# martenlienen/bsi

Measured on AMD Instinct MI355X. Metric: images/sec BSI.sample k=128 (DiT, 3x32x32), higher is better.
Workload: dtype bf16

## Files before the change

bsi_amd/csrc/dit_ops.hip:

```cpp
#include <math.h>

#include "common.h"
#include "dit_ops.h"

namespace {

constexpr int TPB = 256;

__global__ void silu_bf16_kernel(const float* __restrict__ pre, size_t n, __bf16* __restrict__ out) {
    for (size_t i = (size_t)blockIdx.x * blockDim.x + threadIdx.x; i < n; i += (size_t)gridDim.x * blockDim.x)
        out[i] = (__bf16)silu_f(pre[i]);
}

__global__ void cast_bf16_kernel(const float* __restrict__ in, int ld_in, int rows, int cols, __bf16* __restrict__ out, int ld) {
    const int r = blockIdx.y;
    const float* ir = in + (size_t)r * ld_in;
    __bf16* orow = out + (size_t)r * ld;
    for (int c = (blockIdx.x * blockDim.x + threadIdx.x) * 4; c < ld; c += gridDim.x * blockDim.x * 4) {
        float v[4];
#pragma unroll
        for (int k = 0; k < 4; ++k) v[k] = (c + k < cols) ? ir[c + k] : 0.0f;
        if (c + 3 < ld) {
            u32x2 w;
            w[0] = pack_bf16x2(v[0], v[1]);
// ... 185 lines not shown
        const float rstd = 1.0f / sqrtf(wave_sum(q) / (float)d + eps);
        __bf16* orow = out + (size_t)r * d;
#pragma unroll
        for (int i = 0; i < VPL; ++i) {
            const int c = i * 64 + lane;
            if (c < d4) {
                f32x4 y;
#pragma unroll
                for (int k = 0; k < 4; ++k) y[k] = (R.v[i][k] - mean) * rstd;
                const f32x4 a = tab[2][c];
                const f32x4 b = tab[3][c];
#pragma unroll
                for (int k = 0; k < 4; ++k) y[k] = __fmaf_rn(b[k] + 1.0f, y[k], a[k]);
                u32x2 w;
                w[0] = pack_bf16x2(y[0], y[1]);
                w[1] = pack_bf16x2(y[2], y[3]);
                reinterpret_cast<u32x2*>(orow)[c] = w;
            }
        }
    };
    Row A, B;
    if (row >= M) return;
    load(row, A);
    while (true) {
        if (row + stride < M) load(row + stride, B);
        finish(row, A);
        row += stride;
        if (row >= M) break;
        if (row + stride < M) load(row + stride, A);
        finish(row, B);
        row += stride;
        if (row >= M) break;
    }
}

__global__ void fourier_features_kernel(const float* __restrict__ x, size_t total, int C, int inner, int nmin,
                                        int nfreq, float* __restrict__ out) {
    for (size_t idx = (size_t)blockIdx.x * blockDim.x + threadIdx.x; idx < total; idx += (size_t)gridDim.x * blockDim.x) {
        const size_t in_i = idx % inner;
        const size_t oc = idx / inner;
        const float v = x[idx];
        float* o = out + (oc * nfreq * 2) * inner + in_i;
        for (int n = 0; n < nfreq; ++n) {
            const float coef = 6.283185307179586f * (float)(1 << (nmin + n));
            o[(size_t)(n * 2 + 0) * inner] = sinf(__fmaf_rn(coef, v, 0.0f));
            o[(size_t)(n * 2 + 1) * inner] = sinf(__fmaf_rn(coef, v, 1.5707963267948966f));
        }
    }
}

__global__ void dit_prologue_kernel(const float* __restrict__ mu, const float* __restrict__ c_in, int coef_stride, int B,
                                    int C, int H, int W, int ps, int nmin, int nfreq, int kpad, __bf16* __restrict__ out) {
    const int HW = H * W;
    const size_t total = (size_t)B * HW;
    const int Cin = C + C * nfreq * 2;
    const int nw = W / ps;
    const int tokens = (H / ps) * nw;
    const int K = ps * ps * Cin;
    for (size_t idx = (size_t)blockIdx.x * blockDim.x + threadIdx.x; idx < total; idx += (size_t)gridDim.x * blockDim.x) {
        const int b = (int)(idx / HW);
        const int pix = (int)(idx % HW);
        const int h = pix / W, w = pix % W;
        const float ci = c_in ? c_in[(size_t)b * coef_stride] : 1.0f;
        const int tok = (h / ps) * nw + (w / ps);
        const int intra = (h % ps) * ps + (w % ps);
        __bf16* o = out + ((size_t)b * tokens + tok) * kpad + intra * Cin;
        for (int c = 0; c < C; ++c) {
            float v = mu[((size_t)b * C + c) * HW + pix];
            if (c_in) v = __fmul_rn(ci, v);
            o[c] = (__bf16)v;
            for (int n = 0; n < nfreq; ++n) {
                const float coef = 6.283185307179586f * (float)(1 << (nmin + n));
                o[C + (c * nfreq + n) * 2 + 0] = (__bf16)sinf(__fmaf_rn(coef, v, 0.0f));
                o[C + (c * nfreq + n) * 2 + 1] = (__bf16)sinf(__fmaf_rn(coef, v, 1.5707963267948966f));
            }
        }
        if (intra == ps * ps - 1) {
            __bf16* z = out + ((size_t)b * tokens + tok) * kpad;
            for (int c = K; c < kpad; ++c) z[c] = (__bf16)0.0f;
        }
    }
}

template <int VPL, bool WLDS>
__global__ void dit_final_kernel(const float* __restrict__ x, int Mtok, int d, int P, const float* __restrict__ ln_w,
                                 const float* __restrict__ ln_b, const float* __restrict__ dec_w,
                                 const float* __restrict__ dec_b, int C, int H, int W, int ps,
                                 const float* __restrict__ mu, const float* __restrict__ c_skip,
                                 const float* __restrict__ c_out, int coef_stride, const __bf16* __restrict__ delta,
                                 const float* __restrict__ gate, int gate_rows, int gate_stride,
                                 float* __restrict__ out) {
    extern __shared__ __attribute__((aligned(16))) float wsm[];
    const int d4 = d >> 2;
    if constexpr (WLDS) {
        for (int i = threadIdx.x; i < P * d4; i += blockDim.x)
            reinterpret_cast<f32x4*>(wsm)[i] = reinterpret_cast<const f32x4*>(dec_w)[i];
        __syncthreads();
    }
    const int lane = threadIdx.x & 63;
    const int wpb = blockDim.x >> 6;
    const int nw = W / ps;
    const int tokens = (H / ps) * nw;
    const int HW = H * W;
    constexpr int FR = 4;
    for (int row0 = (blockIdx.x * wpb + (threadIdx.x >> 6)) * FR; row0 < Mtok; row0 += gridDim.x * wpb * FR) {
        f32x4 v[FR][VPL];
        float s[FR], q[FR];
#pragma unroll
        for (int r = 0; r < FR; ++r) {
            const int row = row0 + r < Mtok ? row0 + r : Mtok - 1;
            const float* xr = x + (size_t)row * d;
            const int b_idx = row / tokens;
            s[r] = 0.f;
#pragma unroll
            for (int i = 0; i < VPL; ++i) {
                const int c = i * 64 + lane;
                v[r][i] = (c < d4) ? reinterpret_cast<const f32x4*>(xr)[c] : f32x4{0.f, 0.f, 0.f, 0.f};
                if (delta && c < d4) {
                    const u32x2 dw = reinterpret_cast<const u32x2*>(delta + (size_t)row * d)[c];
                    const f32x4 g = reinterpret_cast<const f32x4*>(gate + (size_t)(b_idx % gate_rows) * gate_stride)[c];
                    v[r][i][0] = __fmaf_rn(g[0], __uint_as_float(dw[0] << 16), v[r][i][0]);
                    v[r][i][1] = __fmaf_rn(g[1], __uint_as_float(dw[0] & 0xffff0000u), v[r][i][1]);
                    v[r][i][2] = __fmaf_rn(g[2], __uint_as_float(dw[1] << 16), v[r][i][2]);
                    v[r][i][3] = __fmaf_rn(g[3], __uint_as_float(dw[1] & 0xffff0000u), v[r][i][3]);
                }
                s[r] += (v[r][i][0] + v[r][i][1]) + (v[r][i][2] + v[r][i][3]);
            }
        }
#pragma unroll
        for (int m = 32; m > 0; m >>= 1)
#pragma unroll
            for (int r = 0; r < FR; ++r) s[r] += __shfl_xor(s[r], m, 64);
#pragma unroll
        for (int r = 0; r < FR; ++r) {
            const float mean = s[r] / (float)d;
            s[r] = mean;
            q[r] = 0.f;
#pragma unroll
            for (int i = 0; i < VPL; ++i) {
                const int c = i * 64 + lane;
                if (c < d4) {
#pragma unroll
                    for (int k = 0; k < 4; ++k) {
                        const float dd = v[r][i][k] - mean;
                        q[r] = __fmaf_rn(dd, dd, q[r]);
                    }
                }
            }
        }
#pragma unroll
        for (int m = 32; m > 0; m >>= 1)
#pragma unroll
            for (int r = 0; r < FR; ++r) q[r] += __shfl_xor(q[r], m, 64);
#pragma unroll
        for (int i = 0; i < VPL; ++i) {
            const int c = i * 64 + lane;
            if (c < d4) {
                const f32x4 a = reinterpret_cast<const f32x4*>(ln_w)[c];
                const f32x4 bb = reinterpret_cast<const f32x4*>(ln_b)[c];
#pragma unroll
                for (int r = 0; r < FR; ++r) {
                    const float rstd = 1.0f / sqrtf(q[r] / (float)d + 1e-5f);
#pragma unroll
                    for (int k = 0; k < 4; ++k) v[r][i][k] = __fmaf_rn((v[r][i][k] - s[r]) * rstd, a[k], bb[k]);
                }
            }
        }
        float mine[FR] = {0.f, 0.f, 0.f, 0.f};
        for (int o0 = 0; o0 < P; o0 += 4) {
            float acc[FR][4];
#pragma unroll
            for (int r = 0; r < FR; ++r)
#pragma unroll
                for (int u = 0; u < 4; ++u) acc[r][u] = 0.f;
#pragma unroll
            for (int u = 0; u < 4; ++u) {
                const int o = o0 + u < P ? o0 + u : P - 1;
#pragma unroll
                for (int i = 0; i < VPL; ++i) {
                    const int c = i * 64 + lane;
                    if (c < d4) {
                        const f32x4 wv = WLDS ? reinterpret_cast<const f32x4*>(wsm + (size_t)o * d)[c]
                                              : reinterpret_cast<const f32x4*>(dec_w + (size_t)o * d)[c];
#pragma unroll
                        for (int r = 0; r < FR; ++r)
#pragma unroll
                            for (int k = 0; k < 4; ++k) acc[r][u] = __fmaf_rn(v[r][i][k], wv[k], acc[r][u]);
                    }
                }
            }
#pragma unroll
            for (int m = 32; m > 0; m >>= 1)
#pragma unroll
                for (int r = 0; r < FR; ++r)
#pragma unroll
                    for (int u = 0; u < 4; ++u) acc[r][u] += __shfl_xor(acc[r][u], m, 64);
#pragma unroll
            for (int u = 0; u < 4; ++u)
                if (o0 + u < P && lane == o0 + u) {
#pragma unroll
                    for (int r = 0; r < FR; ++r) mine[r] = acc[r][u] + dec_b[o0 + u];
                }
        }
        if (lane < P) {
            const int intra = lane / C, ch = lane % C;
#pragma unroll
            for (int r = 0; r < FR; ++r) {
                const int row = row0 + r;
                if (row >= Mtok) break;
                const int b_idx = row / tokens, tok = row % tokens;
                const int th = tok / nw, tw = tok % nw;
                const int hh = th * ps + intra / ps, ww = tw * ps + intra % ps;
                const size_t gi = ((size_t)b_idx * C + ch) * HW + (size_t)hh * W + ww;
                float rr = mine[r];
                if (c_skip) {
                    const float cs = c_skip[(size_t)b_idx * coef_stride], co = c_out[(size_t)b_idx * coef_stride];
                    rr = __fmaf_rn(co, mine[r], __fmul_rn(cs, mu[gi]));
                }
                out[gi] = rr;
            }
        }
    }
}

}

#define S(stream) reinterpret_cast<hipStream_t>(stream)

extern "C" int bsi_cast_rows_bf16(const float* in, int ld_in, int rows, int cols, void* out, int ld_out,
                                  bsi_stream_t stream) {
    BSI_CHECK_ARG(in && out && rows > 0 && cols > 0 && ld_in >= cols && ld_out >= cols && ld_out % 4 == 0,
                  "bsi_cast_rows_bf16: bad args rows=%d cols=%d ld_in=%d ld_out=%d", rows, cols, ld_in, ld_out);
    int gx = (ld_out / 4 + TPB - 1) / TPB;
    if (gx > 16) gx = 16;
    hipLaunchKernelGGL(cast_bf16_kernel, dim3(gx, rows), dim3(TPB), 0, S(stream), in, ld_in, rows, cols,
                       reinterpret_cast<__bf16*>(out), ld_out);
    BSI_CHECK_LAUNCH("bsi_cast_bf16");
    return BSI_OK;
}

extern "C" int bsi_cast_bf16(const float* in, int rows, int cols, void* out, int ld_out, bsi_stream_t stream) {
    return bsi_cast_rows_bf16(in, cols, rows, cols, out, ld_out, stream);
}

extern "C" int bsi_silu_bf16(const float* pre, size_t n, void* out, bsi_stream_t stream) {
    BSI_CHECK_ARG(pre && out && n > 0, "bsi_silu_bf16: bad args");
    size_t g = (n + TPB - 1) / TPB;
    if (g > 4096) g = 4096;
    hipLaunchKernelGGL(silu_bf16_kernel, dim3((int)g), dim3(TPB), 0, S(stream), pre, n, reinterpret_cast<__bf16*>(out));
    BSI_CHECK_LAUNCH("bsi_silu_bf16");
    return BSI_OK;
}

extern "C" int bsi_fourier_features(const float* x, int outer, int C, int inner, int n_min, int n_max, float* out,
                                    bsi_stream_t stream) {
    BSI_CHECK_ARG(x && out && outer > 0 && C > 0 && inner > 0 && n_max >= n_min && n_min >= 0 && n_max < 31,
                  "bsi_fourier_features: bad args");
    const size_t total = (size_t)outer * C * inner;
    size_t g = (total + TPB - 1) / TPB;
    if (g > 8192) g = 8192;
    hipLaunchKernelGGL(fourier_features_kernel, dim3((int)g), dim3(TPB), 0, S(stream), x, total, C, inner, n_min,
                       n_max - n_min + 1, out);
    BSI_CHECK_LAUNCH("bsi_fourier_features");
    return BSI_OK;
}

extern "C" int bsi_nyquist_embed(const float* t, int rows, const float* scale, const float* bias, int size,
                                 float* out_f32, void* out_bf16, bsi_stream_t stream) {
    BSI_CHECK_ARG(t && scale && bias && rows > 0 && size > 0 && (out_f32 || out_bf16), "bsi_nyquist_embed: bad args");
    int gx = (size + TPB - 1) / TPB;
    hipLaunchKernelGGL(nyquist_kernel, dim3(gx, rows), dim3(TPB), 0, S(stream), t, rows, scale, bias, size, out_f32,
                       reinterpret_cast<__bf16*>(out_bf16));
    BSI_CHECK_LAUNCH("bsi_nyquist_embed");
    return BSI_OK;
}

int bsi_resid_ln_modulate_drop(float* x, int M, int d, float eps, const void* delta, const float* gate,
                               const float* shift, const float* scale, int mod_rows, int mod_stride, int tokens,
                               const float* ln_w, const float* ln_b, void* out_bf16, DropCfg dc, bsi_stream_t stream,
                               float* x_out, float* stats, const void* delta0, const float* gate0, int write_x, DropCfg mdc,
                               void* maskw) {
    BSI_CHECK_ARG(x && M > 0 && d > 0 && d % 4 == 0 && d <= 2048, "bsi_resid_ln_modulate: bad args M=%d d=%d", M, d);
    BSI_CHECK_ARG(out_bf16 || delta, "bsi_resid_ln_modulate: nothing to do");
    BSI_CHECK_ARG((shift == nullptr) == (scale == nullptr), "bsi_resid_ln_modulate: shift and scale go together");
    BSI_CHECK_ARG((delta == nullptr) == (gate == nullptr), "bsi_resid_ln_modulate: delta and gate go together");
    BSI_CHECK_ARG(!(shift || gate) || (mod_rows > 0 && tokens > 0 && mod_stride % 4 == 0),
                  "bsi_resid_ln_modulate: bad modulation table");
    BSI_CHECK_ARG((ln_w == nullptr) == (ln_b == nullptr), "bsi_resid_ln_modulate: ln weight and bias go together");
    BSI_CHECK_ARG((delta0 == nullptr) == (gate0 == nullptr) && (!delta0 || delta), "bsi_resid_ln_modulate: an older update needs its gate and a newer update");
    BSI_CHECK_ARG(write_x || (delta && out_bf16 && !x_out), "bsi_resid_ln_modulate: write_x = 0 needs an update and an output");
    BSI_CHECK_ARG(!(maskw && mdc.thr) || (d > 256 && d <= 1024 && out_bf16), "bsi_resid_ln_modulate: mask words ride on the d <= 1024 instance");
    const __bf16* dl0 = reinterpret_cast<const __bf16*>(delta0);
    const int wpb = TPB / 64;
    dim3 grid((M + wpb - 1) / wpb);
    __bf16* o = reinterpret_cast<__bf16*>(out_bf16);
    const __bf16* dl = reinterpret_cast<const __bf16*>(delta);
    if (g_bsi_ln_stream_cus > 0 && d > 256 && d <= 1024 && shift && o && mod_rows == 1 && !ln_w && !dc.thr && !x_out && !stats &&
        !(maskw && mdc.thr)) {
        static int per_cu = 0;
        if (per_cu == 0) {
            int n = 0;
            if (hipOccupancyMaxActiveBlocksPerMultiprocessor(&n, ln_modulate_stream_kernel<4>, TPB, 0) != hipSuccess || n < 1) n = 2;
            if (const char* e = getenv("BSI_LN_STREAM_WGS")) n = atoi(e) > 0 ? atoi(e) : n;
            per_cu = n;
        }
        int g = g_bsi_ln_stream_cus * per_cu;
        if (g > (int)grid.x) g = (int)grid.x;
// ... 5 lines not shown
    if (d <= 256)
        hipLaunchKernelGGL(ln_modulate_kernel<1>, grid, dim3(TPB), 0, S(stream), x, M, d, eps, shift, scale, mod_rows,
                           mod_stride, tokens, ln_w, ln_b, dl, gate, o, dc, x_out, stats, dl0, gate0, write_x);
    else if (d <= 1024 && maskw && mdc.thr)
        hipLaunchKernelGGL((ln_modulate_kernel<4, true>), grid, dim3(TPB), 0, S(stream), x, M, d, eps, shift, scale, mod_rows,
                           mod_stride, tokens, ln_w, ln_b, dl, gate, o, dc, x_out, stats, dl0, gate0, write_x, mdc,
                           reinterpret_cast<unsigned long long*>(maskw));
    else if (d <= 1024)
        hipLaunchKernelGGL(ln_modulate_kernel<4>, grid, dim3(TPB), 0, S(stream), x, M, d, eps, shift, scale, mod_rows,
                           mod_stride, tokens, ln_w, ln_b, dl, gate, o, dc, x_out, stats, dl0, gate0, write_x);
    else
        hipLaunchKernelGGL(ln_modulate_kernel<8>, grid, dim3(TPB), 0, S(stream), x, M, d, eps, shift, scale, mod_rows,
                           mod_stride, tokens, ln_w, ln_b, dl, gate, o, dc, x_out, stats, dl0, gate0, write_x);
    BSI_CHECK_LAUNCH("bsi_resid_ln_modulate");
    return BSI_OK;
}

extern "C" int bsi_resid2_ln_modulate(float* x, int M, int d, float eps, const void* delta0, const float* gate0, const void* delta,
                                      const float* gate, int write_x, const float* shift, const float* scale, int mod_rows,
                                      int mod_stride, int tokens, void* out_bf16, bsi_stream_t stream) {
    return bsi_resid_ln_modulate_drop(x, M, d, eps, delta, gate, shift, scale, mod_rows, mod_stride, tokens, nullptr, nullptr,
                                      out_bf16, DropCfg{}, stream, nullptr, nullptr, delta0, gate0, write_x);
}

extern "C" int bsi_resid_ln_modulate(float* x, int M, int d, float eps, const void* delta, const float* gate,
                                     const float* shift, const float* scale, int mod_rows, int mod_stride, int tokens,
                                     const float* ln_w, const float* ln_b, void* out_bf16, bsi_stream_t stream) {
    return bsi_resid_ln_modulate_drop(x, M, d, eps, delta, gate, shift, scale, mod_rows, mod_stride, tokens, ln_w, ln_b,
                                      out_bf16, DropCfg{}, stream);
}

__global__ void dropout_mask_kernel(DropCfg dc, unsigned rows, unsigned cols, uint8_t* __restrict__ out) {
    const size_t n = (size_t)rows * cols;
    for (size_t i = (size_t)blockIdx.x * blockDim.x + threadIdx.x; i < n; i += (size_t)gridDim.x * blockDim.x) {
        const unsigned r = (unsigned)(i / cols), c = (unsigned)(i % cols);
        out[i] = drop_keep_rc(dc, drop_row(dc, r), c) ? 1 : 0;
    }
}

extern "C" int bsi_dropout_mask(float p, unsigned long long seed, unsigned site, unsigned rows, unsigned cols, uint8_t* out,
                                bsi_stream_t stream) {
    BSI_CHECK_ARG(out && rows > 0 && cols > 0 && p >= 0.f && p < 1.f, "bsi_dropout_mask: bad args");
    size_t g = ((size_t)rows * cols + TPB - 1) / TPB;
    if (g > 4096) g = 4096;
    hipLaunchKernelGGL(dropout_mask_kernel, dim3((int)g), dim3(TPB), 0, S(stream), make_drop(p, seed, site), rows, cols, out);
    BSI_CHECK_LAUNCH("bsi_dropout_mask");
    return BSI_OK;
}

extern "C" int bsi_ln_modulate(const float* x, int M, int d, float eps, const float* shift, const float* scale,
                               int mod_rows, int mod_stride, int tokens, const float* ln_w, const float* ln_b,
                               void* out_bf16, bsi_stream_t stream) {
    BSI_CHECK_ARG(out_bf16, "bsi_ln_modulate: null output");
    return bsi_resid_ln_modulate(const_cast<float*>(x), M, d, eps, nullptr, nullptr, shift, scale, mod_rows, mod_stride,
                                 tokens, ln_w, ln_b, out_bf16, stream);
}

int bsi_dit_prologue_launch(const float* mu, const float* c_in, int coef_stride, int B, int C, int H, int W, int ps,
                            int nmin, int nfreq, int kpad, void* out, hipStream_t s) {
    const size_t total = (size_t)B * H * W;
    size_t g = (total + TPB - 1) / TPB;
    if (g > 8192) g = 8192;
    hipLaunchKernelGGL(dit_prologue_kernel, dim3((int)g), dim3(TPB), 0, s, mu, c_in, coef_stride, B, C, H, W, ps, nmin,
                       nfreq, kpad, reinterpret_cast<__bf16*>(out));
    BSI_CHECK_LAUNCH("bsi_dit_prologue");
    return BSI_OK;
}

int bsi_dit_final_launch(const float* x, int Mtok, int d, int P, const float* ln_w, const float* ln_b,
                         const float* dec_w, const float* dec_b, int C, int H, int W, int ps, const float* mu,
                         const float* c_skip, const float* c_out, int coef_stride, const void* delta, const float* gate,
                         int gate_rows, int gate_stride, float* out, hipStream_t s) {
    size_t lds = (size_t)P * d * sizeof(float);
    if (P > 64) {
        bsi_set_error("bsi_dit_final: decoder P=%d unsupported (needs patch*patch*C <= 64)", P);
        return BSI_EINVAL;
    }
    const bool wlds = lds <= 128 * 1024;
    if (!wlds) lds = 0;
    const int wpb = TPB / 64;
    int grid = (Mtok + wpb * 4 - 1) / (wpb * 4);
    if (grid < 1) grid = 1;
    if (grid > 2048) grid = 2048;
#define LAUNCH_FINAL(V)                                                                                              \
    do {                                                                                                             \
        auto kern = wlds ? dit_final_kernel<V, true> : dit_final_kernel<V, false>;                                   \
        (void)hipFuncSetAttribute(reinterpret_cast<const void*>(kern), hipFuncAttributeMaxDynamicSharedMemorySize, (int)lds); \
        hipLaunchKernelGGL(kern, dim3(grid), dim3(TPB), lds, s, x, Mtok, d, P, ln_w, ln_b, dec_w, dec_b, C, H, W, ps, \
                           mu, c_skip, c_out, coef_stride, reinterpret_cast<const __bf16*>(delta), gate,             \
                           gate_rows > 0 ? gate_rows : 1, gate_stride, out);                                         \
    } while (0)
    if (d <= 256) LAUNCH_FINAL(1);
    else if (d <= 1024) LAUNCH_FINAL(4);
    else LAUNCH_FINAL(8);
#undef LAUNCH_FINAL
    BSI_CHECK_LAUNCH("bsi_dit_final");
    return BSI_OK;
}
```

bsi_amd/_native.py:

```python
import ctypes as C
import os

import torch

_HERE = os.path.dirname(os.path.abspath(__file__))
LIB_PATH = os.environ.get("BSI_HIP_LIB") or os.path.join(_HERE, "lib", "libbsi_hip.so")

_lib = None


class BSIParams(C.Structure):
    _fields_ = [("lambda_0", C.c_float), ("alpha_M", C.c_float), ("alpha_R", C.c_float),
                ("ln_low", C.c_float), ("delta", C.c_float)]


class GemmArgs(C.Structure):
    _fields_ = [("A", C.c_void_p), ("W", C.c_void_p), ("bias", C.c_void_p), ("out", C.c_void_p),
                ("M", C.c_int), ("N", C.c_int), ("K", C.c_int),
                ("lda", C.c_int), ("ldw", C.c_int), ("ldo", C.c_int), ("epilogue", C.c_int),
                ("gate", C.c_void_p), ("gate_rows", C.c_int), ("gate_stride", C.c_int),
                ("tokens", C.c_int), ("pos", C.c_void_p), ("aux", C.c_void_p), ("out2", C.c_void_p), ("colsum_rows", C.c_void_p)]


class CastDesc(C.Structure):
# ... 172 lines not shown
    "bsi_attention_fwd": (_i, [_vp, _i, _i, _i, _i, _i, _vp, _i, _vp]),
    "bsi_attention_fwd_lse": (_i, [_vp, _i, _i, _i, _i, _i, _vp, _i, _vp, _vp]),
    "bsi_attention_bwd": (_i, [_vp, _i, _vp, _vp, _i, _vp, _i, _i, _i, _i, _vp, _i, _vp]),
    "bsi_attention_bwd_long": (_i, [_vp, _i, _vp, _vp, _i, _vp, _i, _i, _i, _i, _vp, _i, _vp]),
    "bsi_gate_bwd": (_i, [_vp, _vp, _vp, _vp, _i, _vp, _i, _i, _i, _i, _vp, _vp]),
    "bsi_ln_mod_bwd": (_i, [_vp, _vp, _vp, _i, _vp, _vp, _i, _vp, _i, _i, _i, _f, _vp]),
    "bsi_ln_gate_bwd": (_i, [_vp, _vp, _vp, _vp, _i, _vp, _vp, _i, _vp, _vp, _vp, _i, _vp, _i, _vp, _i, _i, _i, _vp]),
    "bsi_silu_bwd_bf16": (_i, [_vp, _vp, _sz, _vp, _vp]),
    "bsi_cast_transpose_bf16": (_i, [_vp, _i, _i, _vp, _i, _vp]),
    "bsi_cast_batch_tiles": (_i, [_i, _i, _i]),
    "bsi_cast_batch_bf16": (_i, [_vp, _i, _i, _vp]),
    "bsi_cast_rows_bf16": (_i, [_vp, _i, _i, _i, _vp, _i, _vp]),
    "bsi_silu_bf16": (_i, [_vp, _sz, _vp, _vp]),
    "bsi_dit_tape_bytes": (_sz, [C.POINTER(DitConfig), _i]),
    "bsi_dit_backward_workspace_bytes": (_sz, [C.POINTER(DitConfig), _i]),
    "bsi_dit_train_forward": (_i, [C.POINTER(DitConfig), C.POINTER(DitWeights), _i, _vp, _vp, _vp, _vp, _vp, _vp, _vp,
                                   _f, C.c_ulonglong, _vp]),
    "bsi_dit_backward": (_i, [C.POINTER(DitConfig), C.POINTER(DitWeights), C.POINTER(DitWeightsT), C.POINTER(DitGrads), _i,
                              _vp, _vp, _vp, _vp, _f, C.c_ulonglong, _vp]),
    "bsi_dropout_mask": (_i, [_f, C.c_ulonglong, C.c_uint, C.c_uint, C.c_uint, _vp, _vp]),
    "bsi_attention_dropout_words": (_i, [_f, C.c_ulonglong, C.c_uint, _i, _vp, _vp]),
    "bsi_attention_fwd_dropout": (_i, [_vp, _i, _i, _i, _i, _i, _vp, _i, _vp, _f, C.c_ulonglong, C.c_uint, _vp, _vp]),
    "bsi_attention_bwd_dropout": (_i, [_vp, _i, _vp, _vp, _i, _vp, _i, _i, _i, _i, _vp, _i, _f, C.c_ulonglong, C.c_uint, _vp, _vp]),
    "bsi_dit_backward_set_events": (_i, [_vp, _i]),
    "bsi_dit_train_forward_set_gates": (_i, [_vp, _i]),
    "bsi_sqnorm_workspace_bytes": (_sz, []),
    "bsi_grad_sqnorm": (_i, [_vp, _sz, _vp, _vp, _vp]),
    "bsi_clip_adamw_ema": (_i, [_vp, _vp, _vp, _vp, _vp, _sz, _vp, _f, _f, _f, _f, _f, _f, _f, _i, _f, _vp]),
    "bsi_conv_nhwc_bf16": (_i, [C.POINTER(ConvArgs), _vp]),
    "bsi_conv_weight_pack": (_i, [_vp, _i, _i, _i, _i, _i, _i, _vp, _vp]),
    "bsi_conv_weight_pack_t": (_i, [_vp, _i, _i, _i, _i, _vp, _vp]),
    "bsi_conv_weight_pack_batch": (_i, [_vp, _i, _i, _vp]),
    "bsi_conv_wgrad_workspace_bytes": (C.c_size_t, [_i, _i, _i, _i, _i]),
    "bsi_conv_wgrad_nhwc_bf16": (_i, [_vp, _i, _vp, _vp, _vp, _i, _i, _i, _i, _i, _i, _i, _vp, _i, _vp, _vp]),
    "bsi_conv_wgrad_bias_nhwc_bf16": (_i, [_vp, _i, _vp, _vp, _vp, _i, _i, _i, _i, _i, _i, _i, _vp, _vp, _i, _vp, _vp]),
    "bsi_conv_wgrad_unpack": (_i, [_vp, _i, _i, _i, _i, _i, _i, _i, _vp, _vp]),
    "bsi_groupnorm_nhwc": (_i, [_vp, _i, _vp, _i, _i, _i, _vp, _vp, _f, _i, _vp, _vp, _vp]),
    "bsi_groupnorm_stats_nhwc": (_i, [_vp, _i, _vp, _i, _i, _i, _vp, _vp, _f, _i, _vp, _vp, _vp, _vp]),
    "bsi_groupnorm_apply_nhwc": (_i, [_vp, _i, _vp, _vp, _i, _vp, _i, _i, _vp, _vp, _f, _i, _vp, _vp, _vp, _vp]),
    "bsi_groupnorm_bwd_nhwc": (_i, [_vp, _vp, _i, _vp, _i, _i, _i, _vp, _vp, _f, _i, _vp, _vp, _vp, _vp, _vp, _vp, _vp]),
    "bsi_groupnorm_bwd_cast_nhwc": (_i, [_vp, _vp, _i, _vp, _i, _i, _i, _vp, _vp, _f, _i, _vp, _vp, _vp, _vp, _vp, _vp, _vp, _vp, _vp]),
    "bsi_film_silu": (_i, [_vp, _i, _i, _i, _vp, _i, _i, _f, C.c_ulonglong, C.c_uint, _vp, _vp]),
    "bsi_film_silu_bwd": (_i, [_vp, _vp, _i, _i, _i, _vp, _i, _i, _f, C.c_ulonglong, C.c_uint, _vp, _vp, _i, _vp]),
    "bsi_film_act": (_i, [_vp, _i, _i, _i, _vp, _i, _i, _i, _f, C.c_ulonglong, C.c_uint, _vp, _vp]),
    "bsi_film_act_bwd": (_i, [_vp, _vp, _i, _i, _i, _vp, _i, _i, _i, _f, C.c_ulonglong, C.c_uint, _vp, _vp, _i, _vp]),
    "bsi_act_bf16": (_i, [_vp, _sz, _i, _vp, _vp]),
    "bsi_act_bwd_bf16": (_i, [_vp, _vp, _sz, _i, _vp, _vp]),
    "bsi_unet_decode_bwd": (_i, [_vp, _vp, _i, _vp, _i, _i, _i, _vp, _i, _vp, _vp, _vp, _vp]),
    "bsi_unet_decode": (_i, [_vp, _i, _i, _i, _vp, _vp, _i, _vp, _vp, _vp, _i, _vp, _vp]),
    "bsi_unet_cin_pad": (_i, [C.POINTER(UNetConfig)]),
    "bsi_unet_workspace_bytes": (_sz, [C.POINTER(UNetConfig), _i]),
    "bsi_unet_film_scratch_bytes": (_sz, [C.POINTER(UNetConfig), _i]),
    "bsi_unet_film": (_i, [C.POINTER(UNetConfig), C.POINTER(UNetWeights), _vp, _i, _vp, _vp, _vp]),
    "bsi_unet_tape_bytes": (_sz, [C.POINTER(UNetConfig), _i]),
    "bsi_unet_backward_workspace_bytes": (_sz, [C.POINTER(UNetConfig), _i]),
    "bsi_unet_train_forward": (_i, [C.POINTER(UNetConfig), C.POINTER(UNetWeights), _i, _vp, _vp, _vp, _vp, _vp, _vp, _vp, _f,
                                    C.c_ulonglong, _vp]),
    "bsi_unet_backward": (_i, [C.POINTER(UNetConfig), C.POINTER(UNetWeights), C.POINTER(UNetWeightsT), C.POINTER(UNetGrads), _i,
                               _vp, _vp, _vp, _vp, _f, C.c_ulonglong, _vp]),
    "bsi_unet_forward": (_i, [C.POINTER(UNetConfig), C.POINTER(UNetWeights), _i, _vp, _vp, _i, _vp, _vp, _vp, _i, _vp, _vp, _vp]),
    "bsi_dit_kpad": (_i, [C.POINTER(DitConfig)]),
    "bsi_dit_tokens": (_i, [C.POINTER(DitConfig)]),
    "bsi_dit_workspace_bytes": (_sz, [C.POINTER(DitConfig), _i]),
    "bsi_dit_adaln_scratch_bytes": (_sz, [C.POINTER(DitConfig), _i]),
    "bsi_dit_adaln": (_i, [C.POINTER(DitConfig), C.POINTER(DitWeights), _vp, _i, _vp, _vp, _vp]),
    "bsi_dit_forward": (_i, [C.POINTER(DitConfig), C.POINTER(DitWeights), _i, _vp, _vp, _i, _vp, _vp, _vp, _i,
                             _vp, _vp, _vp, _vp]),
    "bsi_cu_pair_create": (_i, [_i, C.POINTER(_vp)]),
    "bsi_cu_pair_destroy": (_i, [_vp]),
    "bsi_cu_pair_streams": (_i, [_vp, C.POINTER(_vp), C.POINTER(_vp), C.POINTER(_i)]),
    "bsi_dit_forward_pair": (_i, [C.POINTER(DitConfig), C.POINTER(DitWeights), _i, _vp, _vp, _i, _vp, _vp, _vp, _i,
                                  _vp, _vp, _vp, _i, _vp]),
    "bsi_sqnorm_segments": (_i, [_vp, _vp, _i, _sz, _vp, _vp]),
    "bsi_sqnorm_finish": (_i, [_vp, _sz, _vp, _vp]),
    "bsi_copy_batch_tiles": (_i, [_sz]),
    "bsi_copy_batch_f32": (_i, [_vp, _i, _i, _vp]),
    "bsi_clip_adamw_ema_segments": (_i, [_vp, _vp, _vp, _vp, _vp, _vp, _i, _sz, _vp, _f, _f, _f, _f, _f, _f, _f, _i, _f, _vp]),
    "bsi_clock_probe": (_i, [_vp, _i, _vp]),
    "bsi_set_cu_reserve": (_i, [_i]),
    "bsi_compute_cus": (_i, []),
    "bsi_set_ln_stream_cus": (_i, [_i]),
    "bsi_set_tile_queue": (_i, [_i]),
    "bsi_set_attention_bwd_skew": (_i, [_i]),
    "bsi_mfma_probe_workspace_bytes": (_sz, []),
    "bsi_mfma_probe": (_i, [_i, _vp, C.POINTER(C.c_int), C.POINTER(C.c_double), _vp]),
    "bsi_prof_enable": (_i, [C.c_uint]),
    "bsi_prof_read": (_i, [_i, C.POINTER(C.c_int), C.POINTER(C.c_double)]),
}

EXPORTS = tuple(_PROTOS)
PROF_CLASSES = {"gemm_qkv": 0, "gemm_out": 1, "gemm_fc1": 2, "gemm_fc2": 3, "attention": 4, "ln_modulate": 5,
                "prologue": 6, "final": 7, "gemm_enc": 8, "adaln": 9}


def fc1_kernel_name():
    return "gemm_bf16_k64r_kernel<BSI_EPI_BIAS_GELU_BF16=2, DYN=false> (fc1)"


def mfma_probe(iters=50000, device=None):
    dev = torch.device(device) if device is not None else torch.device("cuda", torch.cuda.current_device())
    ws = torch.zeros(lib().bsi_mfma_probe_workspace_bytes() // 8, dtype=torch.int64, device=dev)
    nwg, flop = C.c_int(0), C.c_double(0.0)
    check(lib().bsi_mfma_probe(iters, ptr(ws), C.byref(nwg), C.byref(flop), stream()))
    torch.cuda.synchronize(dev)
    w = ws[: 4 * 8 * nwg.value].reshape(nwg.value * 8, 4).cpu()
    ticks = float(int(w[:, 3].max()) - int(w[:, 2].min()))
    return {"tflops": nwg.value * flop.value / (ticks * 1e-8) / 1e12, "mhz": float((100.0 * w[:, 0].double() / w[:, 1].double()).mean()),
            "ms": ticks * 1e-5, "iters": iters}


def prof_enable(names=()):
    mask = 0
    for n in names:
        mask |= 1 << PROF_CLASSES[n]
    check(lib().bsi_prof_enable(mask))


def prof_read(name):
    cnt, tot = C.c_int(0), C.c_double(0.0)
    check(lib().bsi_prof_read(PROF_CLASSES[name], C.byref(cnt), C.byref(tot)))
    return cnt.value, tot.value


def lib():
    global _lib
    if _lib is None:
        if not os.path.isfile(LIB_PATH):
            raise ImportError(
                f"{LIB_PATH} not found: build the HIP extension first "
                "(python -c 'import __graft_entry__ as g; g.build()' or make -C bsi_amd/csrc)")
        _lib = C.CDLL(LIB_PATH)
        for name, (res, args) in _PROTOS.items():
            fn = getattr(_lib, name)
            fn.restype = res
            fn.argtypes = args
        if os.environ.get("BSI_GEMM_VARIANT"):
            _lib.bsi_gemm_set_variant(int(os.environ["BSI_GEMM_VARIANT"]))
        if os.environ.get("BSI_CONV_ABL"):
            _lib.bsi_conv_set_ablation(int(os.environ["BSI_CONV_ABL"]))
    return _lib


def check(rc):
    if rc != 0:
        msg = lib().bsi_last_error()
        raise RuntimeError(f"bsi_hip error {rc}: {msg.decode() if msg else '?'}")


def ptr(t):
    if t is None:
        return None
    if not t.is_cuda:
        raise RuntimeError("bsi_amd: tensor is not on a HIP device; the native path has no CPU fallback")
    if not t.is_contiguous():
        raise RuntimeError("bsi_amd: tensor must be contiguous")
    return C.c_void_p(t.data_ptr())


def stream():
    return C.c_void_p(torch.cuda.current_stream().cuda_stream)
```

include/bsi_hip.h:

```cpp
#ifndef BSI_HIP_H
#define BSI_HIP_H

#include <stddef.h>
#include <stdint.h>

#ifdef __cplusplus
extern "C" {
#endif

typedef void* bsi_stream_t;

enum {
    BSI_OK = 0,
    BSI_EINVAL = -1,
    BSI_ELAUNCH = -2,
    BSI_EUNSUPPORTED = -3,
};

int bsi_version(void);
const char* bsi_last_error(void);


typedef struct bsi_params {
    float lambda_0;
// ... 346 lines not shown
    float* pm1_w_padded; float* pm1_b;
    float* pm3_w; float* pm3_b;
    float* film_w; float* film_b;
    const bsi_unet_resblock_grads* blocks;
    float *agn_w, *agn_b;
    float* aqkv_w; float* aqkv_b;
    float* aout_w; float* aout_b;
} bsi_unet_grads;
size_t bsi_unet_tape_bytes(const bsi_unet_config* cfg, int B);
size_t bsi_unet_backward_workspace_bytes(const bsi_unet_config* cfg, int B);
int bsi_unet_train_forward(const bsi_unet_config* cfg, const bsi_unet_weights* w , int B, const float* mu, const float* t,
                           const float* c_in, const float* c_skip, const float* c_out, float* out, void* tape,
                           float dropout_p, unsigned long long seed, bsi_stream_t stream);
int bsi_unet_backward(const bsi_unet_config* cfg, const bsi_unet_weights* w , const bsi_unet_weights_t* wT ,
                      const bsi_unet_grads* g , int B, const float* g_out, const float* c_out, void* tape,
                      void* workspace, float dropout_p, unsigned long long seed, bsi_stream_t stream);

typedef struct bsi_dit_block_weights_t {
    const void *qkv_wT, *out_wT, *fc1_wT, *fc2_wT, *ada2_wT;
} bsi_dit_block_weights_t;
typedef struct bsi_dit_weights_t {
    const bsi_dit_block_weights_t* blocks;
} bsi_dit_weights_t;

typedef struct bsi_dit_block_grads {
    float *qkv_w, *qkv_b, *out_w, *out_b, *fc1_w, *fc1_b, *fc2_w, *fc2_b, *ada0_w, *ada0_b, *ada2_w, *ada2_b;
} bsi_dit_block_grads;
typedef struct bsi_dit_grads {
    float* enc_w_padded;
    float* enc_b;
    float *dec_ln_w, *dec_ln_b, *dec_w, *dec_b;
    const bsi_dit_block_grads* blocks;
} bsi_dit_grads;

size_t bsi_dit_tape_bytes(const bsi_dit_config* cfg, int B);
size_t bsi_dit_backward_workspace_bytes(const bsi_dit_config* cfg, int B);
int bsi_dit_train_forward(const bsi_dit_config* cfg, const bsi_dit_weights* w , int B, const float* mu,
                          const float* t, const float* c_in, const float* c_skip, const float* c_out, float* out,
                          void* tape, float dropout_p, unsigned long long seed, bsi_stream_t stream);
int bsi_dit_backward(const bsi_dit_config* cfg, const bsi_dit_weights* w , const bsi_dit_weights_t* wT ,
                     const bsi_dit_grads* g , int B, const float* g_out, const float* c_out, void* tape,
                     void* workspace, float dropout_p, unsigned long long seed, bsi_stream_t stream);
int bsi_dropout_mask(float p, unsigned long long seed, unsigned site, unsigned rows, unsigned cols, uint8_t* out ,
                     bsi_stream_t stream);
int bsi_attention_dropout_words(float p, unsigned long long seed, unsigned site, int pairs, void* words, bsi_stream_t stream);
int bsi_attention_fwd_dropout(const void* qkv, int ld_qkv, int B, int tokens, int heads, int dh, void* out, int ld_out, float* lse,
                              float p, unsigned long long seed, unsigned site, void* words, bsi_stream_t stream);
int bsi_attention_bwd_dropout(const void* qkv, int ld_qkv, const void* out, const void* dout, int ld_o, const float* lse, int B,
                              int tokens, int heads, int dh, void* dqkv, int ld_dqkv, float p, unsigned long long seed, unsigned site,
                              const void* words, bsi_stream_t stream);
typedef struct bsi_fwd_gate { void* event; const bsi_cast_desc* cast; int n_cast; int cast_tiles; } bsi_fwd_gate;
int bsi_dit_train_forward_set_gates(const bsi_fwd_gate* gates , int n);
int bsi_dit_backward_set_events(void* const* events, int depth);

size_t bsi_sqnorm_workspace_bytes(void);
int bsi_grad_sqnorm(const float* g, size_t n, float* out_sq, void* workspace, bsi_stream_t stream);
int bsi_clip_adamw_ema(float* p, const float* g, float* m, float* v, float* ema, size_t n, const float* sqnorm,
                       float max_norm, float grad_scale, float lr, float beta1, float beta2, float eps,
                       float weight_decay, int step, float ema_weight, bsi_stream_t stream);

#define BSI_SQNORM_CHUNK 16384
typedef struct bsi_seg {
    size_t p_off, g_off, len, my_chunk, out_chunk;
} bsi_seg;
typedef struct bsi_copy_desc { const float* src; float* dst; size_t len; unsigned tile0, reserved; } bsi_copy_desc;
int bsi_copy_batch_tiles(size_t len);
int bsi_copy_batch_f32(const bsi_copy_desc* descs , int n, int tiles, bsi_stream_t stream);
int bsi_sqnorm_segments(const float* g, const bsi_seg* segs, int nseg, size_t nchunks, float* partials, bsi_stream_t stream);
int bsi_sqnorm_finish(const float* partials, size_t nchunks, float* out_sq, bsi_stream_t stream);
int bsi_clip_adamw_ema_segments(float* p, const float* g, float* m, float* v, float* ema, const bsi_seg* segs, int nseg,
                                size_t nchunks, const float* sqnorm, float max_norm, float grad_scale, float lr, float beta1,
                                float beta2, float eps, float weight_decay, int step, float ema_weight, bsi_stream_t stream);

enum {
    BSI_PROF_GEMM_QKV = 0, BSI_PROF_GEMM_OUT = 1, BSI_PROF_GEMM_FC1 = 2, BSI_PROF_GEMM_FC2 = 3,
    BSI_PROF_ATTN = 4, BSI_PROF_LN = 5, BSI_PROF_PROLOGUE = 6, BSI_PROF_FINAL = 7, BSI_PROF_GEMM_ENC = 8,
    BSI_PROF_ADALN = 9, BSI_PROF_NCLASS = 16
};
#define BSI_MAX_CU_RESERVE 64
int bsi_set_cu_reserve(int cus);
int bsi_compute_cus(void);
int bsi_set_ln_stream_cus(int cus);
int bsi_set_tile_queue(int on);
int bsi_set_attention_bwd_skew(int on);
int bsi_prof_enable(unsigned mask);
int bsi_clock_probe(unsigned long long* out , int us, bsi_stream_t stream);
size_t bsi_mfma_probe_workspace_bytes(void);
int bsi_mfma_probe(int iters, void* workspace, int* workgroups, double* flop_per_workgroup, bsi_stream_t stream);
int bsi_prof_read(int cls, int* count, double* total_ms);

#ifdef __cplusplus
}
#endif
#endif
```

Measured before the change: 46.86.

## Use permlane swap butterfly reduction in DiT final layer decoder

Replaces the per-output full xor-shuffle reductions in the fused final LayerNorm+decoder kernel with a transpose-style butterfly reduction. It uses permlane32/16 swaps and halving steps, so each lane ends up holding one reduced output. Outputs are computed in chunks of 32 accumulators across rows and outputs, with FR adapted to VPL. Delta loads are also hoisted ahead of the gate math, and launch bounds are added. This aims to cut the cross-lane shuffle count, at the cost of more registers and reliance on gfx950 permlane builtins.

```diff
diff --git a/bsi_amd/csrc/dit_ops.hip b/bsi_amd/csrc/dit_ops.hip
--- a/bsi_amd/csrc/dit_ops.hip
+++ b/bsi_amd/csrc/dit_ops.hip
@@ -291,8 +291,23 @@
     }
 }
 
+template <int M, int H, int N>
+__device__ __forceinline__ void halve_step(float (&acc)[N], int lane) {
+    if constexpr (H == 0) {
+        acc[0] += __shfl_xor(acc[0], M, 64);
+    } else {
+        const bool up = (lane & M) != 0;
+#pragma unroll
+        for (int j = 0; j < H; ++j) {
+            const float keep = up ? acc[j + H] : acc[j];
+            const float send = up ? acc[j] : acc[j + H];
+            acc[j] = keep + __shfl_xor(send, M, 64);
+        }
+    }
+}
+
 template <int VPL, bool WLDS>
-__global__ void dit_final_kernel(const float* __restrict__ x, int Mtok, int d, int P, const float* __restrict__ ln_w,
+__global__ __launch_bounds__(TPB) void dit_final_kernel(const float* __restrict__ x, int Mtok, int d, int P, const float* __restrict__ ln_w,
                                  const float* __restrict__ ln_b, const float* __restrict__ dec_w,
                                  const float* __restrict__ dec_b, int C, int H, int W, int ps,
                                  const float* __restrict__ mu, const float* __restrict__ c_skip,
@@ -311,30 +326,48 @@
     const int nw = W / ps;
     const int tokens = (H / ps) * nw;
     const int HW = H * W;
-    constexpr int FR = 4;
+    const bool has1 = delta != nullptr;
+    auto col = [&](int i) { return i * 64 + lane; };
+    auto live = [&](int i) { return i * 64 + lane < d4; };
+    auto gated_update = [&](f32x4& v, const u32x2 dw, const f32x4 g) {
+        v[0] = __fmaf_rn(g[0], __uint_as_float(dw[0] << 16), v[0]);
+        v[1] = __fmaf_rn(g[1], __uint_as_float(dw[0] & 0xffff0000u), v[1]);
+        v[2] = __fmaf_rn(g[2], __uint_as_float(dw[1] << 16), v[2]);
+        v[3] = __fmaf_rn(g[3], __uint_as_float(dw[1] & 0xffff0000u), v[3]);
+    };
+    constexpr int FR = VPL <= 4 ? 4 : 2;
+    constexpr int NV = 32;
+    constexpr int OC = NV / FR;
     for (int row0 = (blockIdx.x * wpb + (threadIdx.x >> 6)) * FR; row0 < Mtok; row0 += gridDim.x * wpb * FR) {
         f32x4 v[FR][VPL];
+        u32x2 db[FR][VPL];
         float s[FR], q[FR];
 #pragma unroll
         for (int r = 0; r < FR; ++r) {
-            const int row = row0 + r < Mtok ? row0 + r : Mtok - 1;
-            const float* xr = x + (size_t)row * d;
-            const int b_idx = row / tokens;
+            const size_t ro = (size_t)min(row0 + r, Mtok - 1) * d;
+#pragma unroll
+            for (int i = 0; i < VPL; ++i) v[r][i] = live(i) ? reinterpret_cast<const f32x4*>(x + ro)[col(i)] : f32x4{0.f, 0.f, 0.f, 0.f};
+        }
+        if (has1) {
+#pragma unroll
+            for (int r = 0; r < FR; ++r) {
+                const size_t ro = (size_t)min(row0 + r, Mtok - 1) * d;
+#pragma unroll
+                for (int i = 0; i < VPL; ++i)
+                    if (live(i)) db[r][i] = reinterpret_cast<const u32x2*>(delta + ro)[col(i)];
+            }
+        }
+#pragma unroll
+        for (int r = 0; r < FR; ++r) {
+            const size_t go = (size_t)((min(row0 + r, Mtok - 1) / tokens) % gate_rows) * gate_stride;
+            if (has1) {
+#pragma unroll
+                for (int i = 0; i < VPL; ++i)
+                    if (live(i)) gated_update(v[r][i], db[r][i], reinterpret_cast<const f32x4*>(gate + go)[col(i)]);
+            }
             s[r] = 0.f;
 #pragma unroll
-            for (int i = 0; i < VPL; ++i) {
-                const int c = i * 64 + lane;
-                v[r][i] = (c < d4) ? reinterpret_cast<const f32x4*>(xr)[c] : f32x4{0.f, 0.f, 0.f, 0.f};
-                if (delta && c < d4) {
-                    const u32x2 dw = reinterpret_cast<const u32x2*>(delta + (size_t)row * d)[c];
-                    const f32x4 g = reinterpret_cast<const f32x4*>(gate + (size_t)(b_idx % gate_rows) * gate_stride)[c];
-                    v[r][i][0] = __fmaf_rn(g[0], __uint_as_float(dw[0] << 16), v[r][i][0]);
-                    v[r][i][1] = __fmaf_rn(g[1], __uint_as_float(dw[0] & 0xffff0000u), v[r][i][1]);
-                    v[r][i][2] = __fmaf_rn(g[2], __uint_as_float(dw[1] << 16), v[r][i][2]);
-                    v[r][i][3] = __fmaf_rn(g[3], __uint_as_float(dw[1] & 0xffff0000u), v[r][i][3]);
-                }
-                s[r] += (v[r][i][0] + v[r][i][1]) + (v[r][i][2] + v[r][i][3]);
-            }
+            for (int i = 0; i < VPL; ++i) s[r] += (v[r][i][0] + v[r][i][1]) + (v[r][i][2] + v[r][i][3]);
         }
 #pragma unroll
         for (int m = 32; m > 0; m >>= 1)
@@ -347,8 +380,7 @@
             q[r] = 0.f;
 #pragma unroll
             for (int i = 0; i < VPL; ++i) {
-                const int c = i * 64 + lane;
-                if (c < d4) {
+                if (live(i)) {
 #pragma unroll
                     for (int k = 0; k < 4; ++k) {
                         const float dd = v[r][i][k] - mean;
@@ -363,10 +395,9 @@
             for (int r = 0; r < FR; ++r) q[r] += __shfl_xor(q[r], m, 64);
 #pragma unroll
         for (int i = 0; i < VPL; ++i) {
-            const int c = i * 64 + lane;
-            if (c < d4) {
-                const f32x4 a = reinterpret_cast<const f32x4*>(ln_w)[c];
-                const f32x4 bb = reinterpret_cast<const f32x4*>(ln_b)[c];
+            if (live(i)) {
+                const f32x4 a = reinterpret_cast<const f32x4*>(ln_w)[col(i)];
+                const f32x4 bb = reinterpret_cast<const f32x4*>(ln_b)[col(i)];
 #pragma unroll
                 for (int r = 0; r < FR; ++r) {
                     const float rstd = 1.0f / sqrtf(q[r] / (float)d + 1e-5f);
@@ -375,56 +406,53 @@
                 }
             }
         }
-        float mine[FR] = {0.f, 0.f, 0.f, 0.f};
-        for (int o0 = 0; o0 < P; o0 += 4) {
-            float acc[FR][4];
-#pragma unroll
-            for (int r = 0; r < FR; ++r)
-#pragma unroll
-                for (int u = 0; u < 4; ++u) acc[r][u] = 0.f;
-#pragma unroll
-            for (int u = 0; u < 4; ++u) {
-                const int o = o0 + u < P ? o0 + u : P - 1;
+        for (int o0 = 0; o0 < P; o0 += OC) {
+            float acc[NV];
+#pragma unroll
+            for (int j = 0; j < NV; ++j) acc[j] = 0.f;
+#pragma unroll
+            for (int u = 0; u < OC; ++u) {
+                int wo = min(o0 + u, P - 1) * d;
+                asm volatile("" : "+s"(wo));
 #pragma unroll
                 for (int i = 0; i < VPL; ++i) {
-                    const int c = i * 64 + lane;
-                    if (c < d4) {
-                        const f32x4 wv = WLDS ? reinterpret_cast<const f32x4*>(wsm + (size_t)o * d)[c]
-                                              : reinterpret_cast<const f32x4*>(dec_w + (size_t)o * d)[c];
-#pragma unroll
-                        for (int r = 0; r < FR; ++r)
-#pragma unroll
-                            for (int k = 0; k < 4; ++k) acc[r][u] = __fmaf_rn(v[r][i][k], wv[k], acc[r][u]);
-                    }
+                    const int cw = min(col(i), d4 - 1);
+                    const f32x4 wv = WLDS ? reinterpret_cast<const f32x4*>(wsm + wo)[cw] : reinterpret_cast<const f32x4*>(dec_w + wo)[cw];
+#pragma unroll
+                    for (int r = 0; r < FR; ++r)
+#pragma unroll
+                        for (int k = 0; k < 4; ++k) acc[r * OC + u] = __fmaf_rn(v[r][i][k], wv[k], acc[r * OC + u]);
                 }
             }
-#pragma unroll
-            for (int m = 32; m > 0; m >>= 1)
-#pragma unroll
-                for (int r = 0; r < FR; ++r)
-#pragma unroll
-                    for (int u = 0; u < 4; ++u) acc[r][u] += __shfl_xor(acc[r][u], m, 64);
-#pragma unroll
-            for (int u = 0; u < 4; ++u)
-                if (o0 + u < P && lane == o0 + u) {
-#pragma unroll
-                    for (int r = 0; r < FR; ++r) mine[r] = acc[r][u] + dec_b[o0 + u];
+            {
+                typedef unsigned u2v __attribute__((ext_vector_type(2)));
+#pragma unroll
+                for (int j = 0; j < NV / 2; ++j) {
+                    const u2v t = __builtin_amdgcn_permlane32_swap(__float_as_uint(acc[j]), __float_as_uint(acc[j + NV / 2]), false, false);
+                    acc[j] = __uint_as_float(t[0]) + __uint_as_float(t[1]);
                 }
-        }
-        if (lane < P) {
-            const int intra = lane / C, ch = lane % C;
-#pragma unroll
-            for (int r = 0; r < FR; ++r) {
-                const int row = row0 + r;
-                if (row >= Mtok) break;
+#pragma unroll
+                for (int j = 0; j < NV / 4; ++j) {
+                    const u2v t = __builtin_amdgcn_permlane16_swap(__float_as_uint(acc[j]), __float_as_uint(acc[j + NV / 4]), false, false);
+                    acc[j] = __uint_as_float(t[0]) + __uint_as_float(t[1]);
+                }
+                halve_step<8, NV / 8>(acc, lane);
+                halve_step<4, NV / 16>(acc, lane);
+                halve_step<2, NV / 32>(acc, lane);
+                halve_step<1, NV / 64>(acc, lane);
+            }
+            const int o = o0 + (lane >> 1) % OC, row = row0 + (lane >> 1) / OC;
+            if ((lane & 1) == 0 && o < P && row < Mtok) {
+                const float f = acc[0] + dec_b[o];
+                const int intra = o / C, ch = o % C;
                 const int b_idx = row / tokens, tok = row % tokens;
                 const int th = tok / nw, tw = tok % nw;
                 const int hh = th * ps + intra / ps, ww = tw * ps + intra % ps;
                 const size_t gi = ((size_t)b_idx * C + ch) * HW + (size_t)hh * W + ww;
-                float rr = mine[r];
+                float rr = f;
                 if (c_skip) {
                     const float cs = c_skip[(size_t)b_idx * coef_stride], co = c_out[(size_t)b_idx * coef_stride];
-                    rr = __fmaf_rn(co, mine[r], __fmul_rn(cs, mu[gi]));
+                    rr = __fmaf_rn(co, f, __fmul_rn(cs, mu[gi]));
                 }
                 out[gi] = rr;
             }
```

After: 46.88, median of 2. Within noise of the previous version (+0.0%).

## Add software-pipelined persistent DiT final-layer kernel with DPP/permlane reductions

Applied to the files above, without the earlier changes.

Adds a persistent final-layer kernel (adaLN gate residual, LayerNorm, decoder projection, unpatchify) whose grid is capped at twice the CU count. Each wave prefetches its next group of rows into registers while it reduces and projects the current group, and LN weights are staged in LDS. Cross-lane sums use permlane swap and DPP butterflies instead of the older reduction. It is enabled by default when d and token counts fit; otherwise the original kernel runs. The cost is extra register pressure, and the final layer is a small part of the whole forward pass.

```diff
diff --git a/bsi_amd/_native.py b/bsi_amd/_native.py
--- a/bsi_amd/_native.py
+++ b/bsi_amd/_native.py
@@ -278,6 +278,7 @@
     "bsi_set_ln_stream_cus": (_i, [_i]),
     "bsi_set_tile_queue": (_i, [_i]),
     "bsi_set_attention_bwd_skew": (_i, [_i]),
+    "bsi_set_dit_final_pipelined": (_i, [_i]),
     "bsi_mfma_probe_workspace_bytes": (_sz, []),
     "bsi_mfma_probe": (_i, [_i, _vp, C.POINTER(C.c_int), C.POINTER(C.c_double), _vp]),
     "bsi_prof_enable": (_i, [C.c_uint]),
diff --git a/bsi_amd/csrc/dit_ops.hip b/bsi_amd/csrc/dit_ops.hip
--- a/bsi_amd/csrc/dit_ops.hip
+++ b/bsi_amd/csrc/dit_ops.hip
@@ -432,6 +432,229 @@
     }
 }
 
+template <int M>
+__device__ __forceinline__ float xor_add(float v) {
+    typedef unsigned u2v __attribute__((ext_vector_type(2)));
+    const int iv = __float_as_int(v);
+    if constexpr (M == 32) {
+        const u2v t = __builtin_amdgcn_permlane32_swap(__float_as_uint(v), __float_as_uint(v), false, false);
+        return __uint_as_float(t[0]) + __uint_as_float(t[1]);
+    } else if constexpr (M == 16) {
+        const u2v t = __builtin_amdgcn_permlane16_swap(__float_as_uint(v), __float_as_uint(v), false, false);
+        return __uint_as_float(t[0]) + __uint_as_float(t[1]);
+    } else if constexpr (M == 8) {
+        return v + __int_as_float(__builtin_amdgcn_update_dpp(0, iv, 0x128, 0xF, 0xF, true));
+    } else if constexpr (M == 4) {
+        const int hm = __builtin_amdgcn_update_dpp(0, iv, 0x141, 0xF, 0xF, true);
+        return v + __int_as_float(__builtin_amdgcn_update_dpp(0, hm, 0x1B, 0xF, 0xF, true));
+    } else if constexpr (M == 2) {
+        return v + __int_as_float(__builtin_amdgcn_update_dpp(0, iv, 0x4E, 0xF, 0xF, true));
+    } else {
+        static_assert(M == 1, "xor_add: lane distance");
+        return v + __int_as_float(__builtin_amdgcn_update_dpp(0, iv, 0xB1, 0xF, 0xF, true));
+    }
+}
+template <int M, int N>
+__device__ __forceinline__ void xor_tree(float (&a)[N]) {
+#pragma unroll
+    for (int j = 0; j < N; ++j) a[j] = xor_add<M>(a[j]);
+    if constexpr (M > 1) xor_tree<M / 2, N>(a);
+}
+
+template <int VPL, bool WLDS, bool FULL, bool DELTA>
+__global__ __launch_bounds__(256, 2) void dit_final_pipe_kernel(const float* __restrict__ x, int Mtok, int d, int P,
+                                                                const float* __restrict__ ln_w, const float* __restrict__ ln_b,
+                                                                const float* __restrict__ dec_w, const float* __restrict__ dec_b,
+                                                                int C, int H, int W, int ps, const float* __restrict__ mu,
+                                                                const float* __restrict__ c_skip, const float* __restrict__ c_out,
+                                                                int coef_stride, const __bf16* __restrict__ delta,
+                                                                const float* __restrict__ gate, int gate_rows, int gate_stride,
+                                                                float* __restrict__ out) {
+    extern __shared__ __attribute__((aligned(16))) float wsm[];
+    const int d4 = d >> 2;
+    f32x4* lnw_s = reinterpret_cast<f32x4*>(wsm);
+    f32x4* lnb_s = lnw_s + VPL * 64;
+    const float* dws = wsm + 2 * VPL * 256;
+    for (int i = threadIdx.x; i < VPL * 64; i += blockDim.x) {
+        const bool in = i < d4;
+        lnw_s[i] = in ? reinterpret_cast<const f32x4*>(ln_w)[i] : f32x4{0.f, 0.f, 0.f, 0.f};
+        lnb_s[i] = in ? reinterpret_cast<const f32x4*>(ln_b)[i] : f32x4{0.f, 0.f, 0.f, 0.f};
+    }
+    if constexpr (WLDS) {
+        for (int i = threadIdx.x; i < P * d4; i += blockDim.x)
+            reinterpret_cast<f32x4*>(wsm + 2 * VPL * 256)[i] = reinterpret_cast<const f32x4*>(dec_w)[i];
+    }
+    __syncthreads();
+    const int lane = threadIdx.x & 63;
+    const int wpb = blockDim.x >> 6;
+    const int nw = W / ps;
+    const int tokens = (H / ps) * nw;
+    const int HW = H * W;
+    constexpr int FR = 4;
+    const int stride = gridDim.x * wpb * FR;
+    int row0 = (blockIdx.x * wpb + (threadIdx.x >> 6)) * FR;
+    if (row0 >= Mtok) return;
+    const float my_b = lane < P ? dec_b[lane] : 0.f;
+
+    f32x4 xr[FR][VPL];
+    u32x2 dr[FR][VPL];
+    auto prefetch = [&](int r0) {
+#pragma unroll
+        for (int r = 0; r < FR; ++r) {
+            const int row = r0 + r;
+#pragma unroll
+            for (int i = 0; i < VPL; ++i) {
+                const int c = i * 64 + lane;
+                const int cc = FULL || c < d4 ? c : 0;
+                xr[r][i] = reinterpret_cast<const f32x4*>(x + (size_t)row * d)[cc];
+                if constexpr (DELTA) dr[r][i] = __builtin_nontemporal_load(reinterpret_cast<const u32x2*>(delta + (size_t)row * d) + cc);
+            }
+        }
+    };
+    prefetch(row0);
+    while (true) {
+        const int b_idx = row0 / tokens;
+        auto pixel = [&](int row) {
+            const int intra = lane / C, ch = lane % C;
+            const int tok = row - b_idx * tokens;
+            const int th = tok / nw, tw = tok % nw;
+            const int hh = th * ps + intra / ps, ww = tw * ps + intra % ps;
+            return ((size_t)b_idx * C + ch) * HW + (size_t)hh * W + ww;
+        };
+        f32x4 gt[VPL];
+#pragma unroll
+        for (int i = 0; i < VPL; ++i) {
+            const int c = i * 64 + lane;
+            gt[i] = f32x4{0.f, 0.f, 0.f, 0.f};
+            if constexpr (DELTA) gt[i] = reinterpret_cast<const f32x4*>(gate + (size_t)(b_idx % gate_rows) * gate_stride)[FULL || c < d4 ? c : 0];
+        }
+        float co = 0.f, skip[FR] = {0.f, 0.f, 0.f, 0.f};
+        if (c_skip && lane < P) {
+            co = c_out[(size_t)b_idx * coef_stride];
+            const float cs = c_skip[(size_t)b_idx * coef_stride];
+#pragma unroll
+            for (int r = 0; r < FR; ++r) skip[r] = __fmul_rn(cs, mu[pixel(row0 + r)]);
+        }
+        f32x4 v[FR][VPL];
+        float s[FR], q[FR];
+#pragma unroll
+        for (int r = 0; r < FR; ++r) s[r] = 0.f;
+#pragma unroll
+        for (int i = 0; i < VPL; ++i) {
+            const int c = i * 64 + lane;
+            const bool in = FULL || c < d4;
+            const f32x4 g = gt[i];
+#pragma unroll
+            for (int r = 0; r < FR; ++r) {
+                v[r][i] = xr[r][i];
+                if constexpr (DELTA) {
+                    const u32x2 dw = dr[r][i];
+                    v[r][i][0] = __fmaf_rn(g[0], __uint_as_float(dw[0] << 16), v[r][i][0]);
+                    v[r][i][1] = __fmaf_rn(g[1], __uint_as_float(dw[0] & 0xffff0000u), v[r][i][1]);
+                    v[r][i][2] = __fmaf_rn(g[2], __uint_as_float(dw[1] << 16), v[r][i][2]);
+                    v[r][i][3] = __fmaf_rn(g[3], __uint_as_float(dw[1] & 0xffff0000u), v[r][i][3]);
+                }
+                if (!in) v[r][i] = f32x4{0.f, 0.f, 0.f, 0.f};
+            }
+        }
+#pragma unroll
+        for (int r = 0; r < FR; ++r)
+#pragma unroll
+            for (int i = 0; i < VPL; ++i) s[r] += (v[r][i][0] + v[r][i][1]) + (v[r][i][2] + v[r][i][3]);
+        const int next0 = row0 + stride;
+        asm volatile("" : "+v"(s[0]), "+v"(s[1]), "+v"(s[2]), "+v"(s[3]), "+v"(co), "+v"(skip[0]), "+v"(skip[1]), "+v"(skip[2]), "+v"(skip[3]));
+        __builtin_amdgcn_sched_barrier(0);
+        if (next0 < Mtok) prefetch(next0);
+        __builtin_amdgcn_sched_barrier(0);
+        xor_tree<32>(s);
+#pragma unroll
+        for (int r = 0; r < FR; ++r) {
+            const float mean = s[r] / (float)d;
+            s[r] = mean;
+            q[r] = 0.f;
+#pragma unroll
+            for (int i = 0; i < VPL; ++i) {
+                const int c = i * 64 + lane;
+                if (FULL || c < d4) {
+#pragma unroll
+                    for (int k = 0; k < 4; ++k) {
+                        const float dd = v[r][i][k] - mean;
+                        q[r] = __fmaf_rn(dd, dd, q[r]);
+                    }
+                }
+            }
+        }
+        xor_tree<32>(q);
+#pragma unroll
+        for (int i = 0; i < VPL; ++i) {
+            const int c = i * 64 + lane;
+            if (FULL || c < d4) {
+                const f32x4 a = lnw_s[c];
+                const f32x4 bb = lnb_s[c];
+#pragma unroll
+                for (int r = 0; r < FR; ++r) {
+                    const float rstd = 1.0f / sqrtf(q[r] / (float)d + 1e-5f);
+#pragma unroll
+                    for (int k = 0; k < 4; ++k) v[r][i][k] = __fmaf_rn((v[r][i][k] - s[r]) * rstd, a[k], bb[k]);
+                }
+            }
+        }
+        float mine[FR] = {0.f, 0.f, 0.f, 0.f};
+        for (int o0 = 0; o0 < P; o0 += 4) {
+            float acc[FR * 4];
+#pragma unroll
+            for (int j = 0; j < FR * 4; ++j) acc[j] = 0.f;
+#pragma unroll
+            for (int u = 0; u < 4; ++u) {
+                const int o = o0 + u < P ? o0 + u : P - 1;
+#pragma unroll
+                for (int i = 0; i < VPL; ++i) {
+                    const int c = i * 64 + lane;
+                    if (FULL || c < d4) {
+                        const f32x4 wv = WLDS ? reinterpret_cast<const f32x4*>(dws + (size_t)o * d)[c]
+                                              : reinterpret_cast<const f32x4*>(dec_w + (size_t)o * d)[c];
+#pragma unroll
+                        for (int r = 0; r < FR; ++r)
+#pragma unroll
+                            for (int k = 0; k < 4; ++k) acc[r * 4 + u] = __fmaf_rn(v[r][i][k], wv[k], acc[r * 4 + u]);
+                    }
+                }
+            }
+            xor_tree<32>(acc);
+#pragma unroll
+            for (int u = 0; u < 4; ++u)
+                if (o0 + u < P && lane == o0 + u) {
+#pragma unroll
+                    for (int r = 0; r < FR; ++r) mine[r] = acc[r * 4 + u] + my_b;
+                }
+        }
+        if (lane < P) {
+#pragma unroll
+            for (int r = 0; r < FR; ++r) {
+                out[pixel(row0 + r)] = c_skip ? __fmaf_rn(co, mine[r], skip[r]) : mine[r];
+            }
+        }
+        if (next0 >= Mtok) break;
+        row0 = next0;
+    }
+}
+
+template <int VPL>
+auto pick_final_pipe(bool wlds, bool full, bool has_delta) {
+#define PICK(W, F) (has_delta ? dit_final_pipe_kernel<VPL, W, F, true> : dit_final_pipe_kernel<VPL, W, F, false>)
+    if constexpr (VPL == 1) return wlds ? (full ? PICK(true, true) : PICK(true, false)) : (full ? PICK(false, true) : PICK(false, false));
+    else return wlds ? PICK(true, true) : PICK(false, true);
+#undef PICK
+}
+
+}
+
+thread_local int g_bsi_dit_final_pipelined = 1;
+
+extern "C" int bsi_set_dit_final_pipelined(int on) {
+    BSI_CHECK_ARG(on == 0 || on == 1, "bsi_set_dit_final_pipelined: %d is not 0 or 1", on);
+    g_bsi_dit_final_pipelined = on;
+    return BSI_OK;
 }
 
 #define S(stream) reinterpret_cast<hipStream_t>(stream)
@@ -603,7 +826,27 @@
     int grid = (Mtok + wpb * 4 - 1) / (wpb * 4);
     if (grid < 1) grid = 1;
     if (grid > 2048) grid = 2048;
-#define LAUNCH_FINAL(V)                                                                                              \
+    if (g_bsi_dit_final_pipelined && d % 4 == 0 && (d <= 256 || d == 1024) && ((H / ps) * (W / ps)) % 4 == 0 && Mtok % 4 == 0 && (!delta || gate)) {
+        const int vpl = d <= 256 ? 1 : 4;
+        const size_t plds = lds + (size_t)2 * vpl * 256 * sizeof(float);
+        int pgrid = (Mtok + wpb * 4 - 1) / (wpb * 4);
+        if (pgrid > 2 * compute_cus()) pgrid = 2 * compute_cus();
+        if (pgrid < 1) pgrid = 1;
+#define LAUNCH_FINAL_PIPE(V)                                                                                         \
+    do {                                                                                                             \
+        auto kern = pick_final_pipe<V>(wlds, d == V * 256, delta != nullptr);                                        \
+        (void)hipFuncSetAttribute(reinterpret_cast<const void*>(kern), hipFuncAttributeMaxDynamicSharedMemorySize, (int)plds); \
+        hipLaunchKernelGGL(kern, dim3(pgrid), dim3(TPB), plds, s, x, Mtok, d, P, ln_w, ln_b, dec_w, dec_b, C, H, W, ps, \
+                           mu, c_skip, c_out, coef_stride, reinterpret_cast<const __bf16*>(delta), gate,             \
+                           gate_rows > 0 ? gate_rows : 1, gate_stride, out);                                         \
+    } while (0)
+        if (vpl == 1) LAUNCH_FINAL_PIPE(1);
+        else LAUNCH_FINAL_PIPE(4);
+#undef LAUNCH_FINAL_PIPE
+        BSI_CHECK_LAUNCH("bsi_dit_final");
+        return BSI_OK;
+    }
+#define LAUNCH_FINAL(V)                                                                                         \
     do {                                                                                                             \
         auto kern = wlds ? dit_final_kernel<V, true> : dit_final_kernel<V, false>;                                   \
         (void)hipFuncSetAttribute(reinterpret_cast<const void*>(kern), hipFuncAttributeMaxDynamicSharedMemorySize, (int)lds); \
diff --git a/include/bsi_hip.h b/include/bsi_hip.h
--- a/include/bsi_hip.h
+++ b/include/bsi_hip.h
@@ -452,6 +452,7 @@
 int bsi_compute_cus(void);
 int bsi_set_ln_stream_cus(int cus);
 int bsi_set_tile_queue(int on);
+int bsi_set_dit_final_pipelined(int on);
 int bsi_set_attention_bwd_skew(int on);
 int bsi_prof_enable(unsigned mask);
 int bsi_clock_probe(unsigned long long* out , int us, bsi_stream_t stream);
```

Result: no change. 49.00 before, 49.13 after, median of 6 (+0.3%).
